# voutcn/megahit

Hardware: NVIDIA H100
Metric: sorted (k+1)-mer edges/sec at k=27 on 150bp reads (higher is better)
Workload: dtype u32

## Files before the change

megahit_b200/csrc/mhb_count.cuh:

```cuda
#pragma once
#include "mhb.h"
#include "mhb_kernels.cuh"

namespace mhb {

static constexpr int kReadsPerBatch = 64;
static constexpr int kStageWords = 4096;
static constexpr int kExtractThreads = 256;

struct ReadsView {
  const u32 *bin;
  u64 bin_words;
  u64 n_reads;
  u32 fixed_len;
  u32 fixed_stride;
  const u64 *rec_off;
  const u64 *edge_off;
  __device__ __forceinline__ u64 rec_start(u64 r) const { return fixed_len ? r * fixed_stride : rec_off[r]; }
};

template <class F>
__device__ __forceinline__ void for_each_read(const ReadsView &rv, F &&f) {
  __shared__ __align__(16) u32 s_stage[2][kStageWords];
  __shared__ __align__(8) u64 s_bar[2];
  const u32 tid = threadIdx.x, warp = tid >> 5;
  constexpr int NW = kExtractThreads / 32;
  const u64 n_batches = (rv.n_reads + kReadsPerBatch - 1) / kReadsPerBatch;
  if (tid == 0) {
    mbar_init(&s_bar[0], 1);
    mbar_init(&s_bar[1], 1);
    mbar_fence_init();
  }
  __syncthreads();

  auto geom = [&](u64 b, u64 &r0, u64 &r1, u64 &a0, u64 &a1) {
    r0 = b * kReadsPerBatch;
    r1 = r0 + kReadsPerBatch < rv.n_reads ? r0 + kReadsPerBatch : rv.n_reads;
    const u64 w0 = rv.rec_start(r0);
    const u64 w1 = r1 < rv.n_reads ? rv.rec_start(r1) : rv.bin_words;
    a0 = w0 & ~3ull;
    a1 = (w1 + 3) & ~3ull;
  };
  auto issue = [&](u64 b, int st) {
    u64 r0, r1, a0, a1;
    geom(b, r0, r1, a0, a1);
    if (a1 - a0 <= (u64)kStageWords && tid == 0) {
      const u32 bytes = (u32)(a1 - a0) * 4;
      mbar_expect_tx(&s_bar[st], bytes);
      bulk_g2s(&s_stage[st][0], rv.bin + a0, bytes, &s_bar[st]);
    }
  };

  u32 parity[2] = {0, 0};
  u64 b = blockIdx.x;
  int st = 0;
  if (b < n_batches) issue(b, 0);
  for (; b < n_batches; b += gridDim.x, st ^= 1) {
    const u64 nb = b + gridDim.x;
    if (nb < n_batches) issue(nb, st ^ 1);
    u64 r0, r1, a0, a1;
    geom(b, r0, r1, a0, a1);
    const bool staged = (a1 - a0) <= (u64)kStageWords;
    if (staged) {
      mbar_wait(&s_bar[st], parity[st]);
      parity[st] ^= 1;
    }
    for (u64 r = r0 + warp; r < r1; r += NW) {
      const u64 w = rv.rec_start(r);
      const u32 *rec = staged ? &s_stage[st][w - a0] : rv.bin + w;
      const u32 L = rec[0];
      f(r, rec + 1, div_ceil(L, 16), L);
    }
    __syncthreads();
  }
}

template <int W, int WR>
__global__ void __launch_bounds__(kExtractThreads)
    k_count_extract(ReadsView rv, u32 k, u32 *__restrict__ records, u64 *hist, int hist_byte) {
  __shared__ u32 s_hist[256];
  for (int i = threadIdx.x; i < 256; i += kExtractThreads) s_hist[i] = 0;
  const u32 lane = lane_id();
  const u32 K1 = k + 1;
// ... 60 lines not shown
  const u32 lane = lane_id();
  const u32 lt_mask = lanemask_lt();
  const u32 K1 = k + 1;
  for_each_read(rv, [&](u64 r, const u32 *s, u32 nwords, u32 L) {
    if (L < K1) {
      if (!WRITE && lane == 0) per_read[r] = 0;
      return;
    }
    const u32 n_e = L - k;
    u64 run = WRITE ? per_read[r] : 0ull;
    for (u32 q0 = 0; q0 < n_e; q0 += 32) {
      const u32 q = q0 + lane;
      u32 rec[WR], strand;
      bool in = false;
      if (q < n_e) {
        make_count_record<W, WR>(s, nwords, L, k, q, rec, strand);
        const u32 top = rec[0] >> 16;
        in = top >= lo && top <= hi;
      }
      const u32 mask = __ballot_sync(0xffffffffu, in);
      if (in) {
        if constexpr (WRITE) st_rec<WR>(records, run + __popc(mask & lt_mask), rec);
        if (hist) atomicAdd(&s_hist[rec_byte<WR>(rec, hist_byte)], 1u);
      }
      run += __popc(mask);
    }
    if (!WRITE && lane == 0) per_read[r] = run;
  });
  __syncthreads();
  if (hist)
    for (int i = threadIdx.x; i < 256; i += kExtractThreads)
      if (s_hist[i]) atomicAdd((unsigned long long *)&hist[i], (unsigned long long)s_hist[i]);
}

template <int WR>
__device__ __forceinline__ bool same_edge(const u32 (&a)[WR], const u32 (&b)[WR]) {
  bool eq = true;
#pragma unroll
  for (int j = 0; j < WR; ++j) {
    const u32 m = (j == WR - 1) ? ~63u : ~0u;
    eq = eq && ((a[j] & m) == (b[j] & m));
  }
  return eq;
}

static constexpr int kMulHistSmem = 1024;

static __global__ void __launch_bounds__(1024) k_scan_u64(u64 *v, u64 nb, u64 *total_out) {
  __shared__ u64 s_w[33];
  __shared__ u64 s_carry;
  if (threadIdx.x == 0) s_carry = 0;
  __syncthreads();
  const u32 lane = lane_id(), warp = threadIdx.x >> 5;
  for (u64 base = 0; base < nb; base += 1024) {
    const u64 i = base + threadIdx.x;
    const u64 x = i < nb ? v[i] : 0;
    u64 inc = x;
#pragma unroll
    for (int d = 1; d < 32; d <<= 1) {
      u64 t = __shfl_up_sync(0xffffffffu, inc, d);
      if (lane >= (u32)d) inc += t;
    }
    if (lane == 31) s_w[warp] = inc;
    __syncthreads();
    if (warp == 0) {
      u64 w = s_w[lane], winc = w;
#pragma unroll
      for (int d = 1; d < 32; d <<= 1) {
        u64 t = __shfl_up_sync(0xffffffffu, winc, d);
        if (lane >= (u32)d) winc += t;
      }
      s_w[lane] = winc - w;
      if (lane == 31) s_w[32] = winc;
    }
    __syncthreads();
    if (i < nb) v[i] = s_carry + s_w[warp] + inc - x;
    __syncthreads();
    if (threadIdx.x == 0) s_carry += s_w[32];
    __syncthreads();
  }
  if (threadIdx.x == 0 && total_out) *total_out = s_carry;
}

__host__ __device__ inline u64 tipset_capacity(u64 n_tip) {
  u64 c = 1024;
  while (c < 2 * n_tip) c <<= 1;
  return c;
}
__host__ __device__ inline u64 tipset_filter_words(u64 n_tip) {
  u64 c = 1024;
  while (c < n_tip) c <<= 1;
  return c;
}

template <int W>
__device__ __forceinline__ u32 hash_key(const u32 (&key)[W]) {
  u32 h = 0x9E3779B1u;
#pragma unroll
  for (int j = 0; j < W; ++j) {
    h = (h ^ key[j]) * 0x85EBCA77u;
    h ^= h >> 15;
  }
  h *= 0x2C1B3C6Du;
  return h ^ (h >> 13);
}
__device__ __forceinline__ u32 hash2(u32 h) {
  h *= 0xC2B2AE3Du;
  return h ^ (h >> 16);
}

static __global__ void k_count_tips(const uint8_t *aux, u64 n, unsigned long long *out) {
  u64 c = 0;
  for (u64 i = (u64)blockIdx.x * blockDim.x + threadIdx.x; i < n; i += (u64)gridDim.x * blockDim.x)
    c += aux[i] != 0;
  for (int d = 16; d; d >>= 1) c += __shfl_xor_sync(0xffffffffu, c, d);
  if (lane_id() == 0 && c) atomicAdd(out, (unsigned long long)c);
}

template <int W>
__global__ void k_tipset_insert(const u32 *__restrict__ edges, const uint8_t *__restrict__ aux, u64 n, u32 k,
                                u32 *filter, u64 filter_words, u32 *table, u64 cap) {
  const u64 i = (u64)blockIdx.x * blockDim.x + threadIdx.x;
  if (i >= n || aux[i] == 0) return;
  const u32 WE = words_per_edge(k);
  u32 key[W];
#pragma unroll
  for (int j = 0; j < W; ++j) {
    const u32 keep = 2 * (k + 1) - 32 * j;
    key[j] = edges[i * WE + j] & top_mask(keep > 32 ? 32 : keep);
  }
  const u32 h = hash_key<W>(key);
  const u32 fb = hash2(h) & (u32)(filter_words * 32 - 1);
  atomicOr(&filter[fb >> 5], 1u << (fb & 31));
  u64 slot = h & (cap - 1);
  while (true) {
    u32 *e = table + slot * (W + 1);
    if (atomicCAS(e, 0u, (u32)aux[i]) == 0u) {
#pragma unroll
      for (int j = 0; j < W; ++j) e[1 + j] = key[j];
      return;
    }
    slot = (slot + 1) & (cap - 1);
  }
}

static constexpr int kMercyUnroll = 4;

template <int W, int WR>
__global__ void __launch_bounds__(256)
    k_mark_mercy(ReadsView rv, u32 k, const u32 *__restrict__ filter, u64 filter_words, const u32 *__restrict__ table,
                 u64 cap, u32 *first_0_out, u32 *last_0_in) {
  const u32 lane = lane_id();
  const u32 K1 = k + 1;
  const u32 fmask = (u32)(filter_words * 32 - 1);
  for (u64 r = (u64)blockIdx.x * 8 + (threadIdx.x >> 5); r < rv.n_reads; r += (u64)gridDim.x * 8) {
    const u32 *rec0 = rv.bin + rv.rec_start(r);
    const u32 L = rec0[0];
    const u32 *s = rec0 + 1;
    const u32 nwords = div_ceil(L, 16);
    u32 first = 0xFFFFFFFFu;
    long long last = -1;
    if (L >= K1) {
      const u32 n_e = L - k;
      for (u32 q0 = 0; q0 < n_e; q0 += 32 * kMercyUnroll) {
        u32 key[kMercyUnroll][W], strand[kMercyUnroll], fw[kMercyUnroll], h[kMercyUnroll];
        bool live[kMercyUnroll];
#pragma unroll
        for (int u = 0; u < kMercyUnroll; ++u) {
          const u32 q = q0 + 32 * u + lane;
          live[u] = q < n_e;
          h[u] = 0;
          fw[u] = 0;
          strand[u] = 0;
          if (live[u]) {
            u32 rec[WR];
            make_count_record<W, WR>(s, nwords, L, k, q, rec, strand[u]);
#pragma unroll
            for (int j = 0; j < W; ++j) {
              const u32 keep = 2 * K1 - 32 * j;
              key[u][j] = rec[j] & top_mask(keep > 32 ? 32 : keep);
            }
            h[u] = hash_key<W>(key[u]);
            fw[u] = filter[(hash2(h[u]) & fmask) >> 5];
          }
        }
#pragma unroll
        for (int u = 0; u < kMercyUnroll; ++u) {
          if (!live[u] || !((fw[u] >> (hash2(h[u]) & 31)) & 1u)) continue;
          u64 slot = h[u] & (cap - 1);
          u32 flags = 0;
          while (true) {
            const u32 *e = table + slot * (W + 1);
            const u32 f = e[0];
            if (f == 0) break;
            bool eq = true;
#pragma unroll
            for (int j = 0; j < W; ++j) eq = eq && e[1 + j] == key[u][j];
            if (eq) {
              flags = f;
              break;
            }
            slot = (slot + 1) & (cap - 1);
          }
          if (flags) {
            const u32 off = L - K1 - (q0 + 32 * u + lane);
            const bool to_last = ((flags & 1u) && strand[u] == 0) || ((flags & 2u) && strand[u] == 1);
            const bool to_first = ((flags & 1u) && strand[u] == 1) || ((flags & 2u) && strand[u] == 0);
            if (to_last) last = last > (long long)off ? last : (long long)off;
            if (to_first) first = first < off + 1 ? first : off + 1;
          }
        }
      }
    }
    for (int d = 16; d; d >>= 1) {
      const u32 f2 = __shfl_xor_sync(0xffffffffu, first, d);
      const long long l2 = __shfl_xor_sync(0xffffffffu, last, d);
      first = first < f2 ? first : f2;
      last = last > l2 ? last : l2;
    }
    if (lane == 0) {
      first_0_out[r] = first;
      last_0_in[r] = last < 0 ? 0xFFFFFFFFu : (u32)last;
    }
  }
}

static __global__ void __launch_bounds__(256)
    k_mark_mercy_roll(ReadsView rv, u32 k, const u32 *__restrict__ filter, u64 filter_words, const u32 *__restrict__ table,
                      u64 cap, u32 *first_0_out, u32 *last_0_in) {
  constexpr int W = 2;
  const u32 lane = lane_id();
  const u32 K1 = k + 1;
  const u32 fmask = (u32)(filter_words * 32 - 1);
  for (u64 r = (u64)blockIdx.x * 8 + (threadIdx.x >> 5); r < rv.n_reads; r += (u64)gridDim.x * 8) {
    const u32 *rec0 = rv.bin + rv.rec_start(r);
    const u32 L = rec0[0];
    const u32 *s = rec0 + 1;
    const u32 nwords = div_ceil(L, 16);
    u32 first = 0xFFFFFFFFu;
    long long last = -1;
    if (L >= K1) {
      const u32 n_e = L - k;
      for (u32 q0 = 0; q0 < n_e; q0 += 128) {
        const u32 q = q0 + 4 * lane;
        u32 key[4][W], strand[4] = {0, 0, 0, 0}, fw[4] = {0, 0, 0, 0}, h[4] = {0, 0, 0, 0};
        bool live[4] = {false, false, false, false};
        if (q < n_e) {
          u64 rec[4];
          make_count_records_roll<4>(s, nwords, L, k, q, rec, strand);
#pragma unroll
          for (int u = 0; u < 4; ++u) {
            live[u] = q + u < n_e;
            key[u][0] = (u32)(rec[u] >> 32);
            key[u][1] = (u32)rec[u] & ~63u;
            if (live[u]) {
              h[u] = hash_key<W>(key[u]);
              fw[u] = filter[(hash2(h[u]) & fmask) >> 5];
            }
          }
        }
#pragma unroll
        for (int u = 0; u < 4; ++u) {
          if (!live[u] || !((fw[u] >> (hash2(h[u]) & 31)) & 1u)) continue;
          u64 slot = h[u] & (cap - 1);
          u32 flags = 0;
          while (true) {
            const u32 *e = table + slot * (W + 1);
            const u32 f = e[0];
            if (f == 0) break;
            if (e[1] == key[u][0] && e[2] == key[u][1]) {
              flags = f;
              break;
            }
            slot = (slot + 1) & (cap - 1);
          }
          if (flags) {
            const u32 off = L - K1 - (q + u);
            const bool to_last = ((flags & 1u) && strand[u] == 0) || ((flags & 2u) && strand[u] == 1);
            const bool to_first = ((flags & 1u) && strand[u] == 1) || ((flags & 2u) && strand[u] == 0);
            if (to_last) last = last > (long long)off ? last : (long long)off;
            if (to_first) first = first < off + 1 ? first : off + 1;
          }
        }
      }
    }
    for (int d = 16; d; d >>= 1) {
      const u32 f2 = __shfl_xor_sync(0xffffffffu, first, d);
      const long long l2 = __shfl_xor_sync(0xffffffffu, last, d);
      first = first < f2 ? first : f2;
      last = last > l2 ? last : l2;
    }
    if (lane == 0) {
      first_0_out[r] = first;
      last_0_in[r] = last < 0 ? 0xFFFFFFFFu : (u32)last;
    }
  }
}


}

namespace mhb {

static constexpr int kCount3Warps = 8;
__host__ __device__ constexpr int count3_ipl(int wr) { return wr <= 4 ? 16 : (wr <= 8 ? 8 : 4); }
__host__ __device__ constexpr int count3_lane_stride(int wr) {
  return count3_ipl(wr) * wr + (wr == 2 ? 2 : (wr == 4 ? 4 : ((count3_ipl(wr) * wr) % 2 == 0 ? 1 : 0)));
}
__host__ __device__ constexpr int count3_warp_words(int wr) {
  return 32 * count3_lane_stride(wr) + ((wr + 3) & ~3)  + 32 * count3_ipl(wr) ;
}

__device__ __forceinline__ u64 spread16(u64 packed8) {
  return (packed8 & 0xFFull) | ((packed8 & 0xFF00ull) << 8) | ((packed8 & 0xFF0000ull) << 16) |
         ((packed8 & 0xFF000000ull) << 24);
}

struct Tally {
  u32 cnt;
  u64 p, n;
};

template <int WR>
__global__ void __launch_bounds__(kCount3Warps * 32)
    k_count_lanes(const u32 *__restrict__ recs, u64 n, u32 k, int m, u32 n_chunks, u32 *ticket,
                  uint2 *__restrict__ solid_list ,
                  u32 *__restrict__ chunk_count, u64 *mul_hist) {
  constexpr int IPL = count3_ipl(WR), CH = 32 * IPL, LS = count3_lane_stride(WR);
  extern __shared__ __align__(16) u32 smem_w[];
  __shared__ u32 s_hist[kMulHistSmem];
  const u32 lane = lane_id(), warp = threadIdx.x >> 5;
  u32 *s_rec = smem_w + (size_t)warp * count3_warp_words(WR);
  u32 *s_prev = s_rec + 32 * LS;
  u32 *s_info = s_prev + ((WR + 3) & ~3);
  (void)k;
  for (int i = threadIdx.x; i < kMulHistSmem; i += kCount3Warps * 32) s_hist[i] = 0;
  __syncthreads();
  u32 n_ones = 0;

  auto judge = [&](u32 cnt, const u32 (&tp)[4], const u32 (&tn)[4]) -> u32 {
    const u32 c16 = cnt > 65535u ? 65535u : cnt;
    if (c16 == 1u) ++n_ones;
    else if (c16 < (u32)kMulHistSmem) atomicAdd(&s_hist[c16], 1u);
    else atomicAdd((unsigned long long *)&mul_hist[c16], 1ull);
    u32 word = 1u | (c16 << 8);
    if ((long long)cnt >= (long long)m) {
      bool has_in = false, has_out = false;
#pragma unroll
      for (int c = 0; c < 4; ++c) {
        has_in = has_in || (long long)tp[c] >= (long long)m;
        has_out = has_out || (long long)tn[c] >= (long long)m;
      }
      word |= 2u | (has_in ? 0u : 4u) | (has_out ? 0u : 8u);
    }
    return word;
  };

  while (true) {
    u32 chunk = 0;
    if (lane == 0) chunk = atomicAdd(ticket, 1u);
    chunk = __shfl_sync(0xffffffffu, chunk, 0);
    if (chunk >= n_chunks) break;
    const u64 a = (u64)chunk * CH;
    const u64 b = a + CH < n ? a + CH : n;
    const u32 n_here = (u32)(b - a);

#pragma unroll
    for (int i = 0; i < IPL; ++i) {
      const u32 t = (u32)i * 32 + lane;
      if (t < n_here) {
        u32 r[WR];
        ld_rec<WR>(recs, a + t, r);
        u32 *dst = s_rec + (t / IPL) * LS + (t % IPL) * WR;
        if constexpr (WR == 2) *reinterpret_cast<uint2 *>(dst) = make_uint2(r[0], r[1]);
        else if constexpr (WR == 4) *reinterpret_cast<uint4 *>(dst) = make_uint4(r[0], r[1], r[2], r[3]);
        else {
#pragma unroll
          for (int j = 0; j < WR; ++j) dst[j] = r[j];
        }
// ... 282 lines not shown
```

megahit_b200/csrc/mhb_device.cu:

```cuda
#include <cuda_runtime.h>
#include <stdarg.h>
#include <stdio.h>
#include <stdlib.h>
#include <string.h>

#include "mhb.h"
#include "mhb_count.cuh"
#include "mhb_internal.h"
#include "mhb_mercy.cuh"
#include "mhb_s2s.cuh"
#include "mhb_common.cuh"

using namespace mhb;

static thread_local char g_err[1024] = "";
int mhb_set_error(int code, const char *fmt, ...) {
  va_list ap;
  va_start(ap, fmt);
  vsnprintf(g_err, sizeof(g_err), fmt, ap);
  va_end(ap);
  return code;
}
extern "C" const char *mhb_last_error(void) { return g_err; }
extern "C" const char *mhb_version(void) { return "megahit_b200 0.1 (sm_90a; formats of megahit v1.2.9)"; }
// ... 144 lines not shown
#define M2(WW, WRR)                                                                                                   \
  if (W == WW && WR == WRR) {                                                                                         \
    if (write)                                                                                                        \
      k_count_extract_range<WW, WRR, true><<<grid, kExtractThreads, 0, st>>>(rv, k, lo, hi, per_read, records, hist256, hist_byte); \
    else                                                                                                              \
      k_count_extract_range<WW, WRR, false><<<grid, kExtractThreads, 0, st>>>(rv, k, lo, hi, per_read, records, hist256, hist_byte); \
  } else
#define M(WW) M2(WW, WW) M2(WW, WW + 1)
  MHB_FOR_W(M) return mhb_set_error(MHB_ERR_ARG, "unsupported k=%u", k);
#undef M
#undef M2
  CK_LAUNCH();
  if (!write) {
    u64 *bsum = nullptr;
    if (int rc = grow_scratch(((rv.n_reads / kScanTile) + 2) * 8, (void **)&bsum)) return rc;
    if (int rc = scan64(st, per_read, rv.n_reads, total_dev, bsum)) return rc;
    CK(cudaMemcpyAsync(per_read + rv.n_reads, total_dev, 8, cudaMemcpyDeviceToDevice, st));
  }
  return MHB_OK;
}

extern "C" int mhb_count_solid(void *stream, const uint32_t *sorted_records, uint64_t n, uint32_t k, int32_t m,
                               uint32_t *edges_out, uint8_t *aux_out, uint64_t capacity_edges, uint64_t *mul_hist,
                               uint64_t *n_solid_out, void *scratch, size_t scratch_bytes) {
  if (k < 1 || k > MHB_MAX_K || !mul_hist || !n_solid_out) return mhb_set_error(MHB_ERR_ARG, "bad args");
  if (n == 0) return MHB_OK;
  const size_t need = mhb_count_solid_scratch_bytes(n);
  if (scratch_bytes < need) return mhb_set_error(MHB_ERR_ARG, "count scratch too small (%zu < %zu)", scratch_bytes, need);
  cudaStream_t st = (cudaStream_t)stream;
  const u32 WR = count_record_words(k);
  {
#define M(WW)                                                                                                          \
  if (WR == WW) {                                                                                                      \
    constexpr int CH = 32 * count3_ipl(WW);                                                                            \
    const u64 n_chunks = (n + CH - 1) / CH;                                                                            \
    if (n_chunks >= (1ull << 32)) return mhb_set_error(MHB_ERR_ARG, "too many records for one count launch");          \
    const u64 n_sblk = (n_chunks + kScanTile - 1) / kScanTile;                                                         \
    char *p = (char *)scratch;                                                                                         \
    u32 *ticket = (u32 *)p;                                                                                            \
    p += 256;                                                                                                          \
    uint2 *solid_list = (uint2 *)p;                                                                                    \
    p += ((size_t)n_chunks * CH * 8 + 255) & ~(size_t)255;                                                             \
    u32 *chunk_count = (u32 *)p;                                                                                       \
    p += ((size_t)n_chunks * 4 + 255) & ~(size_t)255;                                                                  \
    u64 *chunk_off = (u64 *)p;                                                                                         \
    p += ((size_t)n_chunks * 8 + 255) & ~(size_t)255;                                                                  \
    u64 *bsum = (u64 *)p;                                                                                              \
    CK(cudaMemsetAsync(ticket, 0, 256, st));                                                                           \
    const size_t smem = (size_t)kCount3Warps * count3_warp_words(WW) * 4;                                              \
    static int bps = 0;                                                                                                \
    if (!bps) {                                                                                                        \
      CK(cudaFuncSetAttribute(k_count_lanes<WW>, cudaFuncAttributeMaxDynamicSharedMemorySize, (int)smem));             \
      CK(cudaOccupancyMaxActiveBlocksPerMultiprocessor(&bps, k_count_lanes<WW>, kCount3Warps * 32, smem));             \
      if (bps < 1) bps = 1;                                                                                            \
    }                                                                                                                  \
    u64 grid = (u64)sm_count() * bps;                                                                                  \
    if (grid > (n_chunks + kCount3Warps - 1) / kCount3Warps) grid = (n_chunks + kCount3Warps - 1) / kCount3Warps;      \
    k_count_lanes<WW><<<(unsigned)grid, kCount3Warps * 32, smem, st>>>(sorted_records, n, k, m, (u32)n_chunks, ticket,  \
                                                                      solid_list, chunk_count, mul_hist);             \
    CK_LAUNCH();                                                                                                       \
    k_scan32_sums<<<(unsigned)n_sblk, kScanThreads, 0, st>>>(chunk_count, n_chunks, bsum);                             \
    CK_LAUNCH();                                                                                                       \
    k_scan_u64<<<1, 1024, 0, st>>>(bsum, n_sblk, n_solid_out);                                                         \
    CK_LAUNCH();                                                                                                       \
    k_scan32_apply<<<(unsigned)n_sblk, kScanThreads, 0, st>>>(chunk_count, n_chunks, bsum, chunk_off);                 \
    CK_LAUNCH();                                                                                                       \
    u64 gw = (n_chunks + 7) / 8;                                                                                       \
    if (gw > (u64)sm_count() * 16) gw = (u64)sm_count() * 16;                                                          \
    k_count_write<WW><<<(unsigned)gw, 256, 0, st>>>(sorted_records, k, (u32)n_chunks, solid_list, chunk_count,         \
                                                    chunk_off, edges_out, aux_out, capacity_edges);                   \
  }
    MHB_FOR_WR(M)
#undef M
    CK_LAUNCH();
    return MHB_OK;
  }
  return mhb_set_error(MHB_ERR_ARG, "unsupported k=%u", k);
}

extern "C" size_t mhb_count_solid_scratch_bytes(uint64_t n) {
  return (size_t)(n + 1024) * 8 + (size_t)(n / 128 + 2) * 12 + (size_t)(n / 128 / kScanTile + 2) * 8 + 4096;
}

extern "C" size_t mhb_tipset_bytes(uint64_t n_tip_edges, uint32_t k) {
  return 16 + tipset_filter_words(n_tip_edges) * 4 + tipset_capacity(n_tip_edges) * (size_t)(count_key_words(k) + 1) * 4;
}

static int small_scratch(unsigned long long **out) {
  static unsigned long long *buf[64] = {nullptr};
  int dev = 0;
  CK(cudaGetDevice(&dev));
  if (dev < 0 || dev >= 64) return mhb_set_error(MHB_ERR_CUDA, "device index %d out of range", dev);
  if (!buf[dev]) CK(cudaMalloc((void **)&buf[dev], 256));
  *out = buf[dev];
  return MHB_OK;
}

extern "C" int mhb_count_tip_edges(void *stream, const uint8_t *aux, uint64_t n_solid, uint64_t *n_tip_host) {
  cudaStream_t st = (cudaStream_t)stream;
  unsigned long long *d = nullptr;
  *n_tip_host = 0;
  if (n_solid == 0) return MHB_OK;
  if (int rc = small_scratch(&d)) return rc;
  CK(cudaMemsetAsync(d, 0, 8, st));
  k_count_tips<<<sm_count() * 4, 256, 0, st>>>(aux, n_solid, d);
  CK_LAUNCH();
  CK(cudaMemcpyAsync(n_tip_host, d, 8, cudaMemcpyDeviceToHost, st));
  CK(cudaStreamSynchronize(st));
  return MHB_OK;
}

extern "C" int mhb_tipset_build(void *stream, const uint32_t *edges, const uint8_t *aux, uint64_t n_solid, uint32_t k,
                                void *tipset, size_t tipset_bytes, uint64_t n_tip_edges) {
  if (tipset_bytes < mhb_tipset_bytes(n_tip_edges, k)) return mhb_set_error(MHB_ERR_ARG, "tipset too small");
  cudaStream_t st = (cudaStream_t)stream;
  const u64 hdr[2] = {tipset_capacity(n_tip_edges), tipset_filter_words(n_tip_edges)};
  const u64 cap = hdr[0], fwords = hdr[1];
  CK(cudaMemsetAsync(tipset, 0, mhb_tipset_bytes(n_tip_edges, k), st));
  CK(cudaMemcpyAsync(tipset, hdr, 16, cudaMemcpyHostToDevice, st));
  if (n_solid == 0) return MHB_OK;
  u32 *filter = (u32 *)((char *)tipset + 16);
  u32 *table = filter + fwords;
  const u32 W = count_key_words(k);
  const u64 g = (n_solid + 255) / 256;
#define M(WW) \
  if (W == WW) k_tipset_insert<WW><<<(unsigned)g, 256, 0, st>>>(edges, aux, n_solid, k, filter, fwords, table, cap);
  MHB_FOR_W(M)
#undef M
  CK_LAUNCH();
  return MHB_OK;
}

extern "C" int mhb_count_mark_mercy(void *stream, const mhb_dev_reads *reads, uint32_t k, const void *tipset,
                                    size_t tipset_bytes, uint64_t n_tip_edges, uint32_t *first_0_out,
                                    uint32_t *last_0_in) {
  if (int rc = check_reads(reads, k)) return rc;
  if (reads->n_reads == 0) return MHB_OK;
  if (tipset_bytes < mhb_tipset_bytes(n_tip_edges, k)) return mhb_set_error(MHB_ERR_ARG, "bad tipset");
  cudaStream_t st = (cudaStream_t)stream;
  const ReadsView rv = make_reads_view(reads);
  const u32 W = count_key_words(k), WR = count_record_words(k);
  const u64 cap = tipset_capacity(n_tip_edges), fwords = tipset_filter_words(n_tip_edges);
  const u32 *filter = (const u32 *)((const char *)tipset + 16);
  const u32 *table = filter + fwords;
  u64 g64 = (rv.n_reads + 7) / 8;
  if (g64 > (u64)sm_count() * 16) g64 = (u64)sm_count() * 16;
  const int grid = (int)g64;
  static const bool roll = !(getenv("MHB_EXTRACT_ROLL") && !strcmp(getenv("MHB_EXTRACT_ROLL"), "0"));
  if (roll && W == 2 && WR == 2 && k + 1 >= 17) {
    k_mark_mercy_roll<<<grid, 256, 0, st>>>(rv, k, filter, fwords, table, cap, first_0_out, last_0_in);
    CK_LAUNCH();
    return MHB_OK;
  }
#define M(WW)                                                                                                          \
  if (W == WW && WR == WW)                                                                                             \
    k_mark_mercy<WW, WW><<<grid, 256, 0, st>>>(rv, k, filter, fwords, table, cap, first_0_out, last_0_in);              \
  else if (W == WW && WR == WW + 1)                                                                                    \
    k_mark_mercy<WW, WW + 1><<<grid, 256, 0, st>>>(rv, k, filter, fwords, table, cap, first_0_out, last_0_in);          \
  else
  MHB_FOR_W(M) return mhb_set_error(MHB_ERR_ARG, "unsupported k=%u", k);
#undef M
  CK_LAUNCH();
  return MHB_OK;
}

static SeqsView make_seqs_view(const mhb_dev_seqs *s) {
  SeqsView v;
  v.words = s->words;
  v.n_words = s->n_words;
  v.n_seqs = s->n_seqs;
  v.fixed_len = s->fixed_len;
  v.word_off = s->word_off;
  v.len = s->len;
  v.item_off = s->item_off;
  v.mult = s->mult;
  v.fixed_stride = s->fixed_stride;
  return v;
}

extern "C" int mhb_s2s_extract(void *stream, const mhb_dev_seqs *seqs, uint32_t k, uint32_t *records,
                               uint64_t n_items, uint64_t *hist256, int hist_byte) {
  if (!seqs || k < 9 || k > MHB_MAX_K) return mhb_set_error(MHB_ERR_ARG, "kmer size must be >= 9 and <= 255");
  if (n_items == 0) return MHB_OK;
  if (!seqs->mult && !(seqs->fixed_len && seqs->fixed_stride))
    return mhb_set_error(MHB_ERR_ARG, "seqs->mult is NULL (only allowed for fixed-stride edge records)");
  if (!seqs->fixed_len && (!seqs->word_off || !seqs->len || !seqs->item_off))
    return mhb_set_error(MHB_ERR_ARG, "variable-length sequences need word_off, len and item_off");
  if (seqs->fixed_len && seqs->fixed_len < k + 1) return mhb_set_error(MHB_ERR_ARG, "fixed_len < k+1");
  cudaStream_t st = (cudaStream_t)stream;
  const SeqsView sv = make_seqs_view(seqs);
  const u32 W = s2s_record_words(k);
  if (seqs->fixed_len == k + 1 && seqs->fixed_stride && !seqs->mult && k + 1 <= 32 && k + 1 > 16 &&
      n_items == seqs->n_seqs * 6) {
    u64 ge = (seqs->n_seqs + 255) / 256;
    if (ge > (u64)sm_count() * 32) ge = (u64)sm_count() * 32;
    if (W == 2) k_s2s_extract_edges<2><<<(unsigned)ge, 256, 0, st>>>(seqs->words, seqs->n_seqs, seqs->fixed_stride, k, records, hist256, hist_byte);
    else if (W == 3) k_s2s_extract_edges<3><<<(unsigned)ge, 256, 0, st>>>(seqs->words, seqs->n_seqs, seqs->fixed_stride, k, records, hist256, hist_byte);
    else return mhb_set_error(MHB_ERR_ARG, "internal: unexpected record width %u", W);
    CK_LAUNCH();
    return MHB_OK;
  }
  u64 g = (n_items + 255) / 256;
  if (g > (u64)sm_count() * 32) g = (u64)sm_count() * 32;
#define M(WW) \
  if (W == WW) k_s2s_extract<WW><<<(unsigned)g, 256, 0, st>>>(sv, k, records, n_items, hist256, hist_byte);
  MHB_FOR_WR(M)
#undef M
  CK_LAUNCH();
  return MHB_OK;
}

extern "C" int mhb_s2s_extract_edges_pruned(void *stream, const uint32_t *edges, const uint8_t *aux, uint64_t n_edges,
                                            uint64_t n_with_aux, uint32_t k, uint32_t *records, uint64_t capacity,
                                            uint64_t *cursor_dev, uint64_t *hist256, int hist_byte) {
  if (!edges || (!aux && n_with_aux) || !records || !cursor_dev || k < 9 || k > MHB_MAX_K || n_with_aux > n_edges)
    return mhb_set_error(MHB_ERR_ARG, "bad args");
  if (n_edges == 0) return MHB_OK;
  cudaStream_t st = (cudaStream_t)stream;
  const u32 W = s2s_record_words(k), WE = words_per_edge(k);
  u64 g = (n_edges + 255) / 256;
  if (g > (u64)sm_count() * 32) g = (u64)sm_count() * 32;
#define M(WW)                                                                                                        \
  if (W == WW)                                                                                                       \
    k_s2s_extract_edges_pruned<WW><<<(unsigned)g, 256, 0, st>>>(edges, aux, n_edges, n_with_aux, WE, k, records,       \
                                                               (unsigned long long *)cursor_dev, capacity, hist256, hist_byte);
  MHB_FOR_WR(M)
#undef M
  CK_LAUNCH();
  return MHB_OK;
}

extern "C" int mhb_s2s_extract_range(void *stream, const mhb_dev_seqs *seqs, uint32_t k, uint32_t *records, uint64_t n_items,
                                     uint32_t lo, uint32_t hi, uint64_t *cursor_dev, uint64_t capacity, uint64_t *hist256,
                                     int hist_byte) {
  if (!seqs || k < 9 || k > MHB_MAX_K) return mhb_set_error(MHB_ERR_ARG, "kmer size must be >= 9 and <= 255");
  if (lo > hi || hi > 65535) return mhb_set_error(MHB_ERR_ARG, "bad bucket range [%u, %u]", lo, hi);
  if (records && !cursor_dev) return mhb_set_error(MHB_ERR_ARG, "cursor is NULL");
  if (n_items == 0) return MHB_OK;
  if (!seqs->mult && !(seqs->fixed_len && seqs->fixed_stride))
    return mhb_set_error(MHB_ERR_ARG, "seqs->mult is NULL (only allowed for fixed-stride edge records)");
  if (!seqs->fixed_len && (!seqs->word_off || !seqs->len || !seqs->item_off))
    return mhb_set_error(MHB_ERR_ARG, "variable-length sequences need word_off, len and item_off");
  if (seqs->fixed_len && seqs->fixed_len < k + 1) return mhb_set_error(MHB_ERR_ARG, "fixed_len < k+1");
  cudaStream_t st = (cudaStream_t)stream;
  const SeqsView sv = make_seqs_view(seqs);
  const u32 W = s2s_record_words(k);
// ... 313 lines not shown
```

Measured before the change: 14.24 billion.

## Redesign tip-set filter as shared-memory blocked Bloom with folding and 16B slots

Replaces the single-bit global filter with a multi-bit blocked Bloom filter (one word, 2-3 bits) that is copied into up to 224KB of shared memory per 1024-thread CTA. When the filter is too big, a folded copy is checked first in shared memory and the full one second in global memory. Hash-table slots for W=2 are padded to four words so probes become single uint4 loads, and the rolling kernel gathers its probes in batches. The aim is to cut random global memory traffic and false positives in mercy marking, at the cost of per-block filter loads, an extra fold kernel and lower occupancy.

```diff
diff --git a/megahit_b200/csrc/mhb_count.cuh b/megahit_b200/csrc/mhb_count.cuh
--- a/megahit_b200/csrc/mhb_count.cuh
+++ b/megahit_b200/csrc/mhb_count.cuh
@@ -1,4 +1,7 @@
 #pragma once
+#include <stdlib.h>
+#include <string.h>
+
 #include "mhb.h"
 #include "mhb_kernels.cuh"
 
@@ -225,16 +228,47 @@
   if (threadIdx.x == 0 && total_out) *total_out = s_carry;
 }
 
-__host__ __device__ inline u64 tipset_capacity(u64 n_tip) {
-  u64 c = 1024;
-  while (c < 2 * n_tip) c <<= 1;
-  return c;
-}
-__host__ __device__ inline u64 tipset_filter_words(u64 n_tip) {
-  u64 c = 1024;
-  while (c < n_tip) c <<= 1;
-  return c;
-}
+struct TipsetHeader {
+  u64 capacity;
+  u64 filter_words;
+  u32 fold;
+  u32 filter_bits;
+  u32 resident;
+  u32 reserved;
+};
+static_assert(sizeof(TipsetHeader) == 32, "tip set header");
+static constexpr u64 kTipFilterSmemWords = 224 * 1024 / 4;
+static constexpr u64 kTipMul = 0x9E3779B97F4A7C15ull;
+
+struct TipsetPlan {
+  u64 capacity, filter_words;
+  u32 fold, filter_bits, resident;
+  __host__ __device__ u64 global_words() const { return fold * filter_words; }
+  __host__ __device__ u64 folded_words() const { return fold > 1 ? filter_words : 0; }
+};
+
+inline TipsetPlan tipset_plan(u64 n_tip, const char *spec) {
+  TipsetPlan p;
+  p.capacity = 1024;
+  while (p.capacity < 2 * n_tip) p.capacity <<= 1;
+  char *end = nullptr;
+  const unsigned long long forced = spec && *spec ? strtoull(spec, &end, 10) : 0ull;
+  if (forced > 0 && end && *end == '\0') {
+    p.filter_words = (forced + 3) & ~3ull;
+    p.fold = 1;
+    p.resident = p.filter_words <= kTipFilterSmemWords;
+  } else {
+    const u64 want = ((n_tip + 1) / 2 + 3) & ~3ull;
+    p.filter_words = want < 1024 ? 1024 : (want > kTipFilterSmemWords ? kTipFilterSmemWords : want);
+    p.fold = (u32)((n_tip + p.filter_words - 1) / p.filter_words);
+    if (p.fold < 1) p.fold = 1;
+    p.resident = 3 * n_tip <= 32 * kTipFilterSmemWords && !(spec && !strcmp(spec, "global"));
+  }
+  const u64 probed_words = p.resident ? p.filter_words : p.global_words();
+  p.filter_bits = 32 * probed_words >= 5 * n_tip ? 3 : 2;
+  return p;
+}
+__host__ __device__ constexpr u32 tipset_slot_words(u32 W) { return W == 2 ? 4u : W + 1; }
 
 template <int W>
 __device__ __forceinline__ u32 hash_key(const u32 (&key)[W]) {
@@ -247,9 +281,28 @@
   h *= 0x2C1B3C6Du;
   return h ^ (h >> 13);
 }
-__device__ __forceinline__ u32 hash2(u32 h) {
-  h *= 0xC2B2AE3Du;
-  return h ^ (h >> 16);
+
+__device__ __forceinline__ u64 tip_filter_hash64(u64 key, u32 K1) { return (key >> (64 - 2 * K1)) * kTipMul; }
+template <int W>
+__device__ __forceinline__ u64 tip_filter_hash(const u32 (&key)[W], u32 K1) {
+  if constexpr (W == 1) {
+    return (u64)(key[0] >> (32 - 2 * K1)) * kTipMul;
+  } else if constexpr (W == 2) {
+    return tip_filter_hash64(((u64)key[0] << 32) | key[1], K1);
+  } else {
+    u64 a = 0;
+#pragma unroll
+    for (int j = 0; j < W; j += 2) {
+      a = (a ^ (((u64)key[j] << 32) | (j + 1 < W ? key[j + 1] : 0u))) * kTipMul;
+      a ^= a >> 32;
+    }
+    return a * kTipMul;
+  }
+}
+__device__ __forceinline__ u32 tip_filter_word(u64 h, u32 n_words) { return __umulhi((u32)(h >> 32), n_words); }
+__device__ __forceinline__ u32 tip_filter_mask(u64 h, u32 bits) {
+  const u32 lo = (u32)h;
+  return (1u << (lo >> 27)) | (1u << ((lo >> 22) & 31u)) | (bits > 2 ? 1u << ((lo >> 17) & 31u) : 0u);
 }
 
 static __global__ void k_count_tips(const uint8_t *aux, u64 n, unsigned long long *out) {
@@ -262,22 +315,22 @@
 
 template <int W>
 __global__ void k_tipset_insert(const u32 *__restrict__ edges, const uint8_t *__restrict__ aux, u64 n, u32 k,
-                                u32 *filter, u64 filter_words, u32 *table, u64 cap) {
+                                u32 *filter, TipsetPlan plan, u32 *table) {
   const u64 i = (u64)blockIdx.x * blockDim.x + threadIdx.x;
   if (i >= n || aux[i] == 0) return;
-  const u32 WE = words_per_edge(k);
+  const u32 WE = words_per_edge(k), SW = tipset_slot_words(W);
   u32 key[W];
 #pragma unroll
   for (int j = 0; j < W; ++j) {
     const u32 keep = 2 * (k + 1) - 32 * j;
     key[j] = edges[i * WE + j] & top_mask(keep > 32 ? 32 : keep);
   }
-  const u32 h = hash_key<W>(key);
-  const u32 fb = hash2(h) & (u32)(filter_words * 32 - 1);
-  atomicOr(&filter[fb >> 5], 1u << (fb & 31));
-  u64 slot = h & (cap - 1);
+  const u64 fh = tip_filter_hash<W>(key, k + 1);
+  atomicOr(&filter[tip_filter_word(fh, (u32)plan.global_words())], tip_filter_mask(fh, plan.filter_bits));
+  const u64 cap = plan.capacity;
+  u64 slot = hash_key<W>(key) & (cap - 1);
   while (true) {
-    u32 *e = table + slot * (W + 1);
+    u32 *e = table + slot * SW;
     if (atomicCAS(e, 0u, (u32)aux[i]) == 0u) {
 #pragma unroll
       for (int j = 0; j < W; ++j) e[1 + j] = key[j];
@@ -287,157 +340,244 @@
   }
 }
 
+static __global__ void k_tipset_fold(const u32 *__restrict__ filter, u64 n, u32 fold, u32 *__restrict__ folded) {
+  for (u64 i = (u64)blockIdx.x * blockDim.x + threadIdx.x; i < n; i += (u64)gridDim.x * blockDim.x) {
+    u32 w = 0;
+    for (u32 j = 0; j < fold; ++j) w |= filter[i * fold + j];
+    folded[i] = w;
+  }
+}
+
+static constexpr int kMarkThreads = 1024;
+
+struct TipsetDev {
+  const u32 *filter;
+  const u32 *table;
+  u32 n1, n2, filter_bits;
+  u64 cap;
+  bool smem;
+};
+__device__ __forceinline__ TipsetDev tipset_open(const void *tipset, u32 smem_words, u32 *s_filter) {
+  const TipsetHeader hd = *reinterpret_cast<const TipsetHeader *>(tipset);
+  TipsetPlan p;
+  p.capacity = hd.capacity;
+  p.filter_words = hd.filter_words;
+  p.fold = hd.fold;
+  TipsetDev t;
+  t.filter = reinterpret_cast<const u32 *>((const char *)tipset + sizeof(TipsetHeader));
+  t.table = t.filter + p.global_words() + p.folded_words();
+  t.filter_bits = hd.filter_bits;
+  t.cap = hd.capacity;
+  t.smem = hd.resident && hd.filter_words <= smem_words;
+  t.n1 = t.smem ? (u32)hd.filter_words : (u32)p.global_words();
+  t.n2 = t.smem && hd.fold > 1 ? (u32)p.global_words() : 0u;
+  if (t.smem) {
+    const uint4 *src = reinterpret_cast<const uint4 *>(t.filter + (hd.fold > 1 ? p.global_words() : 0));
+    for (u32 i = threadIdx.x; i < t.n1 / 4; i += blockDim.x) reinterpret_cast<uint4 *>(s_filter)[i] = src[i];
+    __syncthreads();
+  }
+  return t;
+}
+
+__device__ __forceinline__ void mercy_note(u32 flags, u32 strand, u32 off, u32 &first, long long &last) {
+  const bool to_last = ((flags & 1u) && strand == 0) || ((flags & 2u) && strand == 1);
+  const bool to_first = ((flags & 1u) && strand == 1) || ((flags & 2u) && strand == 0);
+  if (to_last) last = last > (long long)off ? last : (long long)off;
+  if (to_first) first = first < off + 1 ? first : off + 1;
+}
+__device__ __forceinline__ void mercy_store(u64 r, u32 first, long long last, u32 *first_0_out, u32 *last_0_in) {
+  for (int d = 16; d; d >>= 1) {
+    const u32 f2 = __shfl_xor_sync(0xffffffffu, first, d);
+    const long long l2 = __shfl_xor_sync(0xffffffffu, last, d);
+    first = first < f2 ? first : f2;
+    last = last > l2 ? last : l2;
+  }
+  if (lane_id() == 0) {
+    first_0_out[r] = first;
+    last_0_in[r] = last < 0 ? 0xFFFFFFFFu : (u32)last;
+  }
+}
+
 static constexpr int kMercyUnroll = 4;
+__host__ __device__ constexpr int mark_threads(int W) { return W <= 3 ? kMarkThreads : 256; }
 
 template <int W, int WR>
-__global__ void __launch_bounds__(256)
-    k_mark_mercy(ReadsView rv, u32 k, const u32 *__restrict__ filter, u64 filter_words, const u32 *__restrict__ table,
-                 u64 cap, u32 *first_0_out, u32 *last_0_in) {
+__global__ void __launch_bounds__(mark_threads(W), 1)
+    k_mark_mercy(ReadsView rv, u32 k, const void *__restrict__ tipset, u32 smem_words, u32 *first_0_out, u32 *last_0_in) {
+  extern __shared__ __align__(16) u32 s_filter[];
+  const TipsetDev ts = tipset_open(tipset, smem_words, s_filter);
+  const u32 lane = lane_id();
+  const u32 K1 = k + 1, SW = tipset_slot_words(W);
+  constexpr u32 NW = mark_threads(W) / 32;
+  auto scan = [&](const u32 *__restrict__ filter) {
+    for (u64 r = (u64)blockIdx.x * NW + (threadIdx.x >> 5); r < rv.n_reads; r += (u64)gridDim.x * NW) {
+      const u32 *rec0 = rv.bin + rv.rec_start(r);
+      const u32 L = rec0[0];
+      const u32 *s = rec0 + 1;
+      const u32 nwords = div_ceil(L, 16);
+      u32 first = 0xFFFFFFFFu;
+      long long last = -1;
+      if (L >= K1) {
+        const u32 n_e = L - k;
+        for (u32 q0 = 0; q0 < n_e; q0 += 32 * kMercyUnroll) {
+          u32 key[kMercyUnroll][W], strand[kMercyUnroll];
+          u64 fh[kMercyUnroll];
+          bool hit[kMercyUnroll];
+#pragma unroll
+          for (int u = 0; u < kMercyUnroll; ++u) {
+            const u32 q = q0 + 32 * u + lane;
+            hit[u] = false;
+            strand[u] = 0;
+            if (q < n_e) {
+              u32 rec[WR];
+              make_count_record<W, WR>(s, nwords, L, k, q, rec, strand[u]);
+#pragma unroll
+              for (int j = 0; j < W; ++j) {
+                const u32 keep = 2 * K1 - 32 * j;
+                key[u][j] = rec[j] & top_mask(keep > 32 ? 32 : keep);
+              }
+              fh[u] = tip_filter_hash<W>(key[u], K1);
+              const u32 mask = tip_filter_mask(fh[u], ts.filter_bits);
+              hit[u] = (filter[tip_filter_word(fh[u], ts.n1)] & mask) == mask;
+            }
+          }
+          if (ts.n2) {
+#pragma unroll
+            for (int u = 0; u < kMercyUnroll; ++u) {
+              const u32 mask = tip_filter_mask(fh[u], ts.filter_bits);
+              if (hit[u]) hit[u] = (ts.filter[tip_filter_word(fh[u], ts.n2)] & mask) == mask;
+            }
+          }
+#pragma unroll
+          for (int u = 0; u < kMercyUnroll; ++u) {
+            if (!hit[u]) continue;
+            u64 slot = hash_key<W>(key[u]) & (ts.cap - 1);
+            u32 flags = 0;
+            while (true) {
+              const u32 *e = ts.table + slot * SW;
+              const u32 f = e[0];
+              if (f == 0) break;
+              bool eq = true;
+#pragma unroll
+              for (int j = 0; j < W; ++j) eq = eq && e[1 + j] == key[u][j];
+              if (eq) {
+                flags = f;
+                break;
+              }
+              slot = (slot + 1) & (ts.cap - 1);
+            }
+            if (flags) mercy_note(flags, strand[u], L - K1 - (q0 + 32 * u + lane), first, last);
+          }
+        }
+      }
+      mercy_store(r, first, last, first_0_out, last_0_in);
+    }
+  };
+  if (ts.smem)
+    scan(s_filter);
+  else
+    scan(ts.filter);
+}
+
+template <int R>
+__device__ __forceinline__ void canon_keys_roll(const u32 *s, u32 nwords, u32 k, u32 q, u64 (&key)[R], u32 (&strand)[R]) {
+  const u32 K1 = k + 1;
+  const u32 T = 64u - 2u * K1;
+  const u32 w0 = q >> 4, sh = (q & 15) * 2;
+  const u32 x0 = s[w0];
+  const u32 x1 = (w0 + 1 < nwords) ? s[w0 + 1] : 0u;
+  const u32 x2 = (w0 + 2 < nwords) ? s[w0 + 2] : 0u;
+  const u32 x3 = (w0 + 3 < nwords) ? s[w0 + 3] : 0u;
+  const u64 S = ((((u64)fshl(x0, x1, sh) << 32) | fshl(x1, x2, sh)) >> T) << T;
+  u64 B = ((~S) >> T) << T;
+  u64 A = (((u64)rev2((u32)S) << 32) | rev2((u32)(S >> 32))) << T;
+  const u32 pi = q + K1;
+  const u32 wa = (pi >> 4) - w0;
+  u32 LA = fshl(wa == 1 ? x1 : x2, wa == 1 ? x2 : x3, (pi & 15) * 2);
+  const u64 lowmask = ~((1ull << T) - 1ull);
+#pragma unroll
+  for (int j = 0; j < R; ++j) {
+    const bool st = B < A;
+    key[j] = st ? B : A;
+    strand[j] = st ? 1u : 0u;
+    const u32 b = LA >> 30;
+    B = (B << 2) | (u64)((3u - b) << T);
+    A = ((A >> 2) & lowmask) | ((u64)b << 62);
+    LA <<= 2;
+  }
+}
+
+static __global__ void __launch_bounds__(kMarkThreads, 1)
+    k_mark_mercy_roll(ReadsView rv, u32 k, const void *__restrict__ tipset, u32 smem_words, u32 *first_0_out,
+                      u32 *last_0_in) {
+  extern __shared__ __align__(16) u32 s_filter[];
+  const TipsetDev ts = tipset_open(tipset, smem_words, s_filter);
   const u32 lane = lane_id();
   const u32 K1 = k + 1;
-  const u32 fmask = (u32)(filter_words * 32 - 1);
-  for (u64 r = (u64)blockIdx.x * 8 + (threadIdx.x >> 5); r < rv.n_reads; r += (u64)gridDim.x * 8) {
-    const u32 *rec0 = rv.bin + rv.rec_start(r);
-    const u32 L = rec0[0];
-    const u32 *s = rec0 + 1;
-    const u32 nwords = div_ceil(L, 16);
-    u32 first = 0xFFFFFFFFu;
-    long long last = -1;
-    if (L >= K1) {
-      const u32 n_e = L - k;
-      for (u32 q0 = 0; q0 < n_e; q0 += 32 * kMercyUnroll) {
-        u32 key[kMercyUnroll][W], strand[kMercyUnroll], fw[kMercyUnroll], h[kMercyUnroll];
-        bool live[kMercyUnroll];
-#pragma unroll
-        for (int u = 0; u < kMercyUnroll; ++u) {
-          const u32 q = q0 + 32 * u + lane;
-          live[u] = q < n_e;
-          h[u] = 0;
-          fw[u] = 0;
-          strand[u] = 0;
-          if (live[u]) {
-            u32 rec[WR];
-            make_count_record<W, WR>(s, nwords, L, k, q, rec, strand[u]);
-#pragma unroll
-            for (int j = 0; j < W; ++j) {
-              const u32 keep = 2 * K1 - 32 * j;
-              key[u][j] = rec[j] & top_mask(keep > 32 ? 32 : keep);
+  constexpr u32 NW = kMarkThreads / 32;
+  const uint4 *table = reinterpret_cast<const uint4 *>(ts.table);
+  auto scan = [&](const u32 *__restrict__ filter) {
+    for (u64 r = (u64)blockIdx.x * NW + (threadIdx.x >> 5); r < rv.n_reads; r += (u64)gridDim.x * NW) {
+      const u32 *rec0 = rv.bin + rv.rec_start(r);
+      const u32 L = rec0[0];
+      const u32 *s = rec0 + 1;
+      const u32 nwords = div_ceil(L, 16);
+      u32 first = 0xFFFFFFFFu;
+      long long last = -1;
+      if (L >= K1) {
+        const u32 n_e = L - k;
+        for (u32 q0 = 0; q0 < n_e; q0 += 128) {
+          const u32 q = q0 + 4 * lane;
+          u64 rec[4];
+          u32 strand[4] = {0, 0, 0, 0};
+          bool hit[4] = {false, false, false, false};
+          if (q < n_e) {
+            canon_keys_roll<4>(s, nwords, k, q, rec, strand);
+#pragma unroll
+            for (int u = 0; u < 4; ++u) {
+              const u64 fh = tip_filter_hash64(rec[u], K1);
+              const u32 mask = tip_filter_mask(fh, ts.filter_bits);
+              hit[u] = q + u < n_e && (filter[tip_filter_word(fh, ts.n1)] & mask) == mask;
             }
-            h[u] = hash_key<W>(key[u]);
-            fw[u] = filter[(hash2(h[u]) & fmask) >> 5];
+          }
+          if (!(hit[0] | hit[1] | hit[2] | hit[3])) continue;
+          if (ts.n2) {
+#pragma unroll
+            for (int u = 0; u < 4; ++u) {
+              const u64 fh = tip_filter_hash64(rec[u], K1);
+              const u32 mask = tip_filter_mask(fh, ts.filter_bits);
+              if (hit[u]) hit[u] = (ts.filter[tip_filter_word(fh, ts.n2)] & mask) == mask;
+            }
+            if (!(hit[0] | hit[1] | hit[2] | hit[3])) continue;
+          }
+          u64 slot[4];
+          uint4 e[4];
+#pragma unroll
+          for (int u = 0; u < 4; ++u) {
+            if (!hit[u]) continue;
+            const u32 key[2] = {(u32)(rec[u] >> 32), (u32)rec[u]};
+            slot[u] = hash_key<2>(key) & (ts.cap - 1);
+            e[u] = table[slot[u]];
+          }
+#pragma unroll
+          for (int u = 0; u < 4; ++u) {
+            if (!hit[u]) continue;
+            const u32 k0 = (u32)(rec[u] >> 32), k1 = (u32)rec[u];
+            while (e[u].x != 0 && !(e[u].y == k0 && e[u].z == k1)) {
+              slot[u] = (slot[u] + 1) & (ts.cap - 1);
+              e[u] = table[slot[u]];
+            }
+            if (e[u].x) mercy_note(e[u].x, strand[u], L - K1 - (q + u), first, last);
           }
         }
-#pragma unroll
-        for (int u = 0; u < kMercyUnroll; ++u) {
-          if (!live[u] || !((fw[u] >> (hash2(h[u]) & 31)) & 1u)) continue;
-          u64 slot = h[u] & (cap - 1);
-          u32 flags = 0;
-          while (true) {
-            const u32 *e = table + slot * (W + 1);
-            const u32 f = e[0];
-            if (f == 0) break;
-            bool eq = true;
-#pragma unroll
-            for (int j = 0; j < W; ++j) eq = eq && e[1 + j] == key[u][j];
-            if (eq) {
-              flags = f;
-              break;
-            }
-            slot = (slot + 1) & (cap - 1);
-          }
-          if (flags) {
-            const u32 off = L - K1 - (q0 + 32 * u + lane);
-            const bool to_last = ((flags & 1u) && strand[u] == 0) || ((flags & 2u) && strand[u] == 1);
-            const bool to_first = ((flags & 1u) && strand[u] == 1) || ((flags & 2u) && strand[u] == 0);
-            if (to_last) last = last > (long long)off ? last : (long long)off;
-            if (to_first) first = first < off + 1 ? first : off + 1;
-          }
-        }
-      }
-    }
-    for (int d = 16; d; d >>= 1) {
-      const u32 f2 = __shfl_xor_sync(0xffffffffu, first, d);
-      const long long l2 = __shfl_xor_sync(0xffffffffu, last, d);
-      first = first < f2 ? first : f2;
-      last = last > l2 ? last : l2;
-    }
-    if (lane == 0) {
-      first_0_out[r] = first;
-      last_0_in[r] = last < 0 ? 0xFFFFFFFFu : (u32)last;
-    }
-  }
-}
-
-static __global__ void __launch_bounds__(256)
-    k_mark_mercy_roll(ReadsView rv, u32 k, const u32 *__restrict__ filter, u64 filter_words, const u32 *__restrict__ table,
-                      u64 cap, u32 *first_0_out, u32 *last_0_in) {
-  constexpr int W = 2;
-  const u32 lane = lane_id();
-  const u32 K1 = k + 1;
-  const u32 fmask = (u32)(filter_words * 32 - 1);
-  for (u64 r = (u64)blockIdx.x * 8 + (threadIdx.x >> 5); r < rv.n_reads; r += (u64)gridDim.x * 8) {
-    const u32 *rec0 = rv.bin + rv.rec_start(r);
-    const u32 L = rec0[0];
-    const u32 *s = rec0 + 1;
-    const u32 nwords = div_ceil(L, 16);
-    u32 first = 0xFFFFFFFFu;
-    long long last = -1;
-    if (L >= K1) {
-      const u32 n_e = L - k;
-      for (u32 q0 = 0; q0 < n_e; q0 += 128) {
-        const u32 q = q0 + 4 * lane;
-        u32 key[4][W], strand[4] = {0, 0, 0, 0}, fw[4] = {0, 0, 0, 0}, h[4] = {0, 0, 0, 0};
-        bool live[4] = {false, false, false, false};
-        if (q < n_e) {
-          u64 rec[4];
-          make_count_records_roll<4>(s, nwords, L, k, q, rec, strand);
-#pragma unroll
-          for (int u = 0; u < 4; ++u) {
-            live[u] = q + u < n_e;
-            key[u][0] = (u32)(rec[u] >> 32);
-            key[u][1] = (u32)rec[u] & ~63u;
-            if (live[u]) {
-              h[u] = hash_key<W>(key[u]);
-              fw[u] = filter[(hash2(h[u]) & fmask) >> 5];
-            }
-          }
-        }
-#pragma unroll
-        for (int u = 0; u < 4; ++u) {
-          if (!live[u] || !((fw[u] >> (hash2(h[u]) & 31)) & 1u)) continue;
-          u64 slot = h[u] & (cap - 1);
-          u32 flags = 0;
-          while (true) {
-            const u32 *e = table + slot * (W + 1);
-            const u32 f = e[0];
-            if (f == 0) break;
-            if (e[1] == key[u][0] && e[2] == key[u][1]) {
-              flags = f;
-              break;
-            }
-            slot = (slot + 1) & (cap - 1);
-          }
-          if (flags) {
-            const u32 off = L - K1 - (q + u);
-            const bool to_last = ((flags & 1u) && strand[u] == 0) || ((flags & 2u) && strand[u] == 1);
-            const bool to_first = ((flags & 1u) && strand[u] == 1) || ((flags & 2u) && strand[u] == 0);
-            if (to_last) last = last > (long long)off ? last : (long long)off;
-            if (to_first) first = first < off + 1 ? first : off + 1;
-          }
-        }
-      }
-    }
-    for (int d = 16; d; d >>= 1) {
-      const u32 f2 = __shfl_xor_sync(0xffffffffu, first, d);
-      const long long l2 = __shfl_xor_sync(0xffffffffu, last, d);
-      first = first < f2 ? first : f2;
-      last = last > l2 ? last : l2;
-    }
-    if (lane == 0) {
-      first_0_out[r] = first;
-      last_0_in[r] = last < 0 ? 0xFFFFFFFFu : (u32)last;
-    }
-  }
+      }
+      mercy_store(r, first, last, first_0_out, last_0_in);
+    }
+  };
+  if (ts.smem)
+    scan(s_filter);
+  else
+    scan(ts.filter);
 }
 
 
diff --git a/megahit_b200/csrc/mhb_device.cu b/megahit_b200/csrc/mhb_device.cu
--- a/megahit_b200/csrc/mhb_device.cu
+++ b/megahit_b200/csrc/mhb_device.cu
@@ -250,8 +250,12 @@
   return (size_t)(n + 1024) * 8 + (size_t)(n / 128 + 2) * 12 + (size_t)(n / 128 / kScanTile + 2) * 8 + 4096;
 }
 
+static TipsetPlan tipset_plan_env(uint64_t n_tip) { return tipset_plan(n_tip, getenv("MHB_TIPSET_FILTER")); }
+
 extern "C" size_t mhb_tipset_bytes(uint64_t n_tip_edges, uint32_t k) {
-  return 16 + tipset_filter_words(n_tip_edges) * 4 + tipset_capacity(n_tip_edges) * (size_t)(count_key_words(k) + 1) * 4;
+  const TipsetPlan p = tipset_plan_env(n_tip_edges);
+  return sizeof(TipsetHeader) + (p.global_words() + p.folded_words()) * 4 +
+         p.capacity * (size_t)tipset_slot_words(count_key_words(k)) * 4;
 }
 
 static int small_scratch(unsigned long long **out) {
@@ -282,19 +286,46 @@
                                 void *tipset, size_t tipset_bytes, uint64_t n_tip_edges) {
   if (tipset_bytes < mhb_tipset_bytes(n_tip_edges, k)) return mhb_set_error(MHB_ERR_ARG, "tipset too small");
   cudaStream_t st = (cudaStream_t)stream;
-  const u64 hdr[2] = {tipset_capacity(n_tip_edges), tipset_filter_words(n_tip_edges)};
-  const u64 cap = hdr[0], fwords = hdr[1];
+  const TipsetPlan plan = tipset_plan_env(n_tip_edges);
+  TipsetHeader hdr;
+  memset(&hdr, 0, sizeof(hdr));
+  hdr.capacity = plan.capacity;
+  hdr.filter_words = plan.filter_words;
+  hdr.fold = plan.fold;
+  hdr.filter_bits = plan.filter_bits;
+  hdr.resident = plan.resident;
   CK(cudaMemsetAsync(tipset, 0, mhb_tipset_bytes(n_tip_edges, k), st));
-  CK(cudaMemcpyAsync(tipset, hdr, 16, cudaMemcpyHostToDevice, st));
+  CK(cudaMemcpyAsync(tipset, &hdr, sizeof(hdr), cudaMemcpyHostToDevice, st));
   if (n_solid == 0) return MHB_OK;
-  u32 *filter = (u32 *)((char *)tipset + 16);
-  u32 *table = filter + fwords;
+  u32 *filter = (u32 *)((char *)tipset + sizeof(TipsetHeader));
+  u32 *table = filter + plan.global_words() + plan.folded_words();
   const u32 W = count_key_words(k);
   const u64 g = (n_solid + 255) / 256;
 #define M(WW) \
-  if (W == WW) k_tipset_insert<WW><<<(unsigned)g, 256, 0, st>>>(edges, aux, n_solid, k, filter, fwords, table, cap);
+  if (W == WW) k_tipset_insert<WW><<<(unsigned)g, 256, 0, st>>>(edges, aux, n_solid, k, filter, plan, table);
   MHB_FOR_W(M)
 #undef M
+  CK_LAUNCH();
+  if (plan.fold > 1) {
+    k_tipset_fold<<<(unsigned)((plan.filter_words + 255) / 256), 256, 0, st>>>(filter, plan.filter_words, plan.fold,
+                                                                              filter + plan.global_words());
+    CK_LAUNCH();
+  }
+  return MHB_OK;
+}
+
+template <class Kernel>
+static int launch_mark(Kernel kern, int threads, const ReadsView &rv, uint32_t k, const void *tipset, u32 smem_words,
+                       uint32_t *first_0_out, uint32_t *last_0_in, cudaStream_t st) {
+  const size_t smem = (size_t)smem_words * 4;
+  CK(cudaFuncSetAttribute(kern, cudaFuncAttributeMaxDynamicSharedMemorySize, (int)smem));
+  int bps = 0;
+  CK(cudaOccupancyMaxActiveBlocksPerMultiprocessor(&bps, kern, threads, smem));
+  if (bps < 1) return mhb_set_error(MHB_ERR_CUDA, "mercy-mark kernel: no CTA of %d threads and %zu B fits an SM", threads, smem);
+  const u64 warps = threads / 32;
+  u64 grid = (u64)sm_count() * bps;
+  if (grid > (rv.n_reads + warps - 1) / warps) grid = (rv.n_reads + warps - 1) / warps;
+  kern<<<(unsigned)grid, threads, smem, st>>>(rv, k, tipset, smem_words, first_0_out, last_0_in);
   CK_LAUNCH();
   return MHB_OK;
 }
@@ -308,28 +339,19 @@
   cudaStream_t st = (cudaStream_t)stream;
   const ReadsView rv = make_reads_view(reads);
   const u32 W = count_key_words(k), WR = count_record_words(k);
-  const u64 cap = tipset_capacity(n_tip_edges), fwords = tipset_filter_words(n_tip_edges);
-  const u32 *filter = (const u32 *)((const char *)tipset + 16);
-  const u32 *table = filter + fwords;
-  u64 g64 = (rv.n_reads + 7) / 8;
-  if (g64 > (u64)sm_count() * 16) g64 = (u64)sm_count() * 16;
-  const int grid = (int)g64;
+  const TipsetPlan plan = tipset_plan_env(n_tip_edges);
+  const u32 smem_words = plan.resident ? (u32)plan.filter_words : 0u;
   static const bool roll = !(getenv("MHB_EXTRACT_ROLL") && !strcmp(getenv("MHB_EXTRACT_ROLL"), "0"));
-  if (roll && W == 2 && WR == 2 && k + 1 >= 17) {
-    k_mark_mercy_roll<<<grid, 256, 0, st>>>(rv, k, filter, fwords, table, cap, first_0_out, last_0_in);
-    CK_LAUNCH();
-    return MHB_OK;
-  }
+  if (roll && W == 2 && WR == 2 && k + 1 >= 17)
+    return launch_mark(k_mark_mercy_roll, kMarkThreads, rv, k, tipset, smem_words, first_0_out, last_0_in, st);
 #define M(WW)                                                                                                          \
   if (W == WW && WR == WW)                                                                                             \
-    k_mark_mercy<WW, WW><<<grid, 256, 0, st>>>(rv, k, filter, fwords, table, cap, first_0_out, last_0_in);              \
+    return launch_mark(k_mark_mercy<WW, WW>, mark_threads(WW), rv, k, tipset, smem_words, first_0_out, last_0_in, st);                   \
   else if (W == WW && WR == WW + 1)                                                                                    \
-    k_mark_mercy<WW, WW + 1><<<grid, 256, 0, st>>>(rv, k, filter, fwords, table, cap, first_0_out, last_0_in);          \
+    return launch_mark(k_mark_mercy<WW, WW + 1>, mark_threads(WW), rv, k, tipset, smem_words, first_0_out, last_0_in, st);               \
   else
   MHB_FOR_W(M) return mhb_set_error(MHB_ERR_ARG, "unsupported k=%u", k);
 #undef M
-  CK_LAUNCH();
-  return MHB_OK;
 }
 
 static SeqsView make_seqs_view(const mhb_dev_seqs *s) {
```

New measurement: 14.75 billion, median of 6. 1.04x the previous value.
